# soasme/LTX-Video-GPUPoor

Measured on AMD Instinct MI355X. Metric: denoise-steps/sec + VAE-decode frames/sec, LTX-Video 768x512x97f at 1/8 GPU, higher is better.
Workload: dtype bf16

## Files before the change

### include/ltxmi.h

```cpp
#ifndef LTXMI_H
#define LTXMI_H

#include <stddef.h>
#include <stdint.h>

#ifdef __cplusplus
extern "C" {
#endif

typedef enum ltxmi_status {
    LTXMI_OK = 0,
    LTXMI_ERR_INVALID_ARG = -1,
    LTXMI_ERR_UNSUPPORTED = -2,
    LTXMI_ERR_LAUNCH = -3
} ltxmi_status;

const char* ltxmi_version(void);
const char* ltxmi_last_error(void);
const char* ltxmi_arch(void);

typedef enum ltxmi_epilogue {
    LTXMI_EPI_NONE = 0,
    LTXMI_EPI_GELU_TANH = 1,
    LTXMI_EPI_SILU = 2,
    LTXMI_EPI_GATE_RESIDUAL = 3
} ltxmi_epilogue;

typedef struct ltxmi_gemm_args {
    const void* A;  int64_t lda;
    const void* W;  int64_t ldw;
    const void* bias;
    void*       C;  int64_t ldc;
    int32_t M, N, K;
    int32_t epilogue;
    const void* residual; int64_t ldr;
    const void* gate_table;
    const void* gate_temb;
    int64_t     gate_ld;
    int32_t     rows_per_group;
    int32_t     algo;
    float*      rowsumsq; int32_t rowsumsq_cols; int64_t rowsumsq_ld;
    int32_t     a_kblock; int64_t a_kblock_stride;
} ltxmi_gemm_args;

int ltxmi_gemm_bf16(const ltxmi_gemm_args* args, void* stream);
int ltxmi_gemm_kernel_id(const ltxmi_gemm_args* args);

typedef enum ltxmi_norm_kind { LTXMI_NORM_RMS = 0, LTXMI_NORM_LAYER = 1 } ltxmi_norm_kind;

int ltxmi_norm_modulate_bf16(const void* x, int64_t ldx, void* y, int64_t ldy,
                             int32_t rows, int32_t D, float eps, int32_t kind,
                             const void* scale_table, const void* scale_temb,
// ... 161 lines not shown
```

### ltx-video-gpupoor_amd/csrc/api.hip

```cpp
#include <stdarg.h>
#include <string.h>

#include "common.h"

namespace ltxmi {

static thread_local char g_err[512] = "";

void set_error(const char* fmt, ...) {
    va_list ap;
    va_start(ap, fmt);
    vsnprintf(g_err, sizeof(g_err), fmt, ap);
    va_end(ap);
}

int check_launch(const char* what) {
    const hipError_t e = hipGetLastError();
    if (e != hipSuccess) {
        set_error("%s: launch failed: %s", what, hipGetErrorString(e));
        return LTXMI_ERR_LAUNCH;
    }
    return LTXMI_OK;
}

// ... 6 lines not shown
    const bool tracked = dev >= 0 && dev < 64;
    const unsigned long long bit = tracked ? (1ull << dev) : 0ull;
    if (tracked && (__atomic_load_n(done, __ATOMIC_ACQUIRE) & bit)) return LTXMI_OK;
    const hipError_t e = hipFuncSetAttribute(kernel, hipFuncAttributeMaxDynamicSharedMemorySize, bytes);
    if (e != hipSuccess) {
        set_error("%s: cannot reserve %d bytes of LDS: %s", what, bytes, hipGetErrorString(e));
        return LTXMI_ERR_LAUNCH;
    }
    if (tracked) __atomic_fetch_or(done, bit, __ATOMIC_RELEASE);
    return LTXMI_OK;
}

int device_cu_count(const char* what) {
    static int cus[64] = {};
    int dev = 0;
    if (hipGetDevice(&dev) != hipSuccess) {
        set_error("%s: cannot query the current device", what);
        return -1;
    }
    const bool tracked = dev >= 0 && dev < 64;
    if (tracked) {
        const int c = __atomic_load_n(&cus[dev], __ATOMIC_ACQUIRE);
        if (c > 0) return c;
    }
    int n = 0;
    if (hipDeviceGetAttribute(&n, hipDeviceAttributeMultiprocessorCount, dev) != hipSuccess || n <= 0) {
        set_error("%s: cannot query the CU count of device %d", what, dev);
        return -1;
    }
    if (tracked) __atomic_store_n(&cus[dev], n, __ATOMIC_RELEASE);
    return n;
}

}

extern "C" const char* ltxmi_version(void) { return "ltxmi 0.9.0"; }
extern "C" const char* ltxmi_last_error(void) { return ltxmi::g_err; }
extern "C" const char* ltxmi_arch(void) { return "gfx950"; }
```

### ltx-video-gpupoor_amd/csrc/attention_cross.hip

```cpp
#include <type_traits>

#include "attention.h"

namespace ltxmi {

namespace cross {

#ifndef LTXMI_XATTN_STAGGER
#define LTXMI_XATTN_STAGGER 32
#endif

constexpr int DH = 64;
constexpr int KV_TILE = 64;
constexpr int MAX_TILES = 4;
constexpr int ROW_BYTES = DH * 2;
constexpr int TILE_BYTES = KV_TILE * DH * 2;
constexpr int K_OFF = 0, V_OFF = MAX_TILES * TILE_BYTES, BIAS_OFF = 2 * MAX_TILES * TILE_BYTES;
constexpr int SCR_OFF = BIAS_OFF + MAX_TILES * KV_TILE * 16;
constexpr int SCR_BYTES = 32 * 64;
constexpr int QW_OFF = SCR_OFF + 4 * SCR_BYTES;
constexpr int SMEM = QW_OFF + DH * 2;
constexpr int ROWS_PER_IT = 128;
constexpr float LOG2E = 1.4426950408889634f;

__device__ __forceinline__ int k_swz(int row) { return (row >> 1) & 7; }

template <int NT>
__global__ __launch_bounds__(256, 2) void attn_cross_kernel(AttnParams p, int groups, int rows_per_group, int stagger_from) {
    extern __shared__ __attribute__((aligned(16))) char smem[];
    const int tid = threadIdx.x;
    const int lane = tid & 63;
    const int wave = __builtin_amdgcn_readfirstlane(tid >> 6);
    const int r = lane & 31, hh = lane >> 5;

    const int work = xcd_work_id();
    const int bh = work / groups, grp = work % groups;
    const int b = bh / p.H, head = bh % p.H;
    const int row_begin = grp * rows_per_group;
    const int row_end = min(p.Lq, row_begin + rows_per_group);
    if (row_begin >= row_end) return;
    const int n_it = (row_end - row_begin + ROWS_PER_IT - 1) / ROWS_PER_IT;

    const uint16_t* qb = p.q + (int64_t)b * p.q_sb + head * DH;
    const uint16_t* kb_ = p.k + (int64_t)b * p.k_sb + head * DH;
    const uint16_t* vb = p.v + (int64_t)b * p.v_sb + head * DH;
    uint16_t* ob = p.o + (int64_t)b * p.o_sb + head * DH;
    constexpr int nt = NT;

    {
        u32x4 kreg[NT][2], vreg[NT][2];
#pragma unroll
        for (int t = 0; t < NT; ++t) {
#pragma unroll
                for (int i = 0; i < 2; ++i) {
                    const int c = tid + 256 * i;
                    int key = t * KV_TILE + (c >> 3);
                    key = key < p.Lk ? key : p.Lk - 1;
                    kreg[t][i] = *(const u32x4*)(kb_ + (int64_t)key * p.k_sl + (c & 7) * 8);
                    vreg[t][i] = *(const u32x4*)(vb + (int64_t)key * p.v_sl + (c & 7) * 8);
                }
            }
// ... 16 lines not shown
                    *(u32x4*)(smem + V_OFF + t * TILE_BYTES + ((key >> 3) * 2 + (dc >> 2)) * 512 + (key & 7) * 64 + (dc & 3) * 16) = vreg[t][i];
                }
            }
    }
    if (p.q_on_load() && tid < 8) *(u32x4*)(smem + QW_OFF + tid * 16) = *(const u32x4*)(p.q_w + head * DH + tid * 8);
    __syncthreads();

    const int k_rd0 = r * ROW_BYTES, k_rd1 = (32 + r) * ROW_BYTES;
    const int k_sw0 = k_swz(r);
    const int g16 = lane >> 4, i16 = lane & 15;
    const int v_rd = (4 * (g16 >> 1) + (i16 >> 2)) * 64 + (16 * (g16 & 1) + 4 * (i16 & 3)) * 2;
    bf16x8 ones;
    {
        const bool on = ((lane & 15) == 0 && ((lane >> 4) & 1) == 0) || ((lane & 15) == 1 && ((lane >> 4) & 1) == 1);
#pragma unroll
        for (int e = 0; e < 8; ++e) ones[e] = on ? (__bf16)1.0f : (__bf16)0.0f;
    }
    const float c = p.scale_log2e;
    char* scr = smem + SCR_OFF + wave * SCR_BYTES;

    bf16x8 qraw[4], qf[4];
    float q_rstd = 0.f;
    int q_ld = 0;
    auto load_q = [&](int it) {
        const int row = row_begin + it * ROWS_PER_IT + wave * 32 + r;
        q_ld = row < p.Lq ? row : p.Lq - 1;
#pragma unroll
        for (int s = 0; s < 4; ++s) qraw[s] = *(const bf16x8*)(qb + (int64_t)q_ld * p.q_sl + 16 * s + 8 * hh);
        if (p.q_on_load()) q_rstd = p.q_row_rstd(b, q_ld, p.H * DH);
    };
    auto finish_q = [&]() {
        if (p.q_on_load()) {
            const int64_t trow = (int64_t)b * p.rope_sb + (int64_t)q_ld * p.rope_sl;
#pragma unroll
            for (int s = 0; s < 4; ++s) {
                const bf16x8 wv = *(const bf16x8*)(smem + QW_OFF + (16 * s + 8 * hh) * 2);
                float o[8];
#pragma unroll
                for (int e = 0; e < 8; ++e) o[e] = (float)qraw[s][e] * q_rstd * (float)wv[e];
                if (p.rope_cos) {
                    const int col = head * DH + 16 * s + 8 * hh;
                    const bf16x8 cv = *(const bf16x8*)(p.rope_cos + trow + col), sv = *(const bf16x8*)(p.rope_sin + trow + col);
#pragma unroll
                    for (int e = 0; e < 8; e += 2) {
                        const float r0 = o[e] * (float)cv[e] - o[e + 1] * (float)sv[e];
                        const float r1 = o[e + 1] * (float)cv[e + 1] + o[e] * (float)sv[e + 1];
                        o[e] = r0;
                        o[e + 1] = r1;
                    }
                }
#pragma unroll
                for (int e = 0; e < 8; ++e) qf[s][e] = (__bf16)o[e];
            }
        } else {
#pragma unroll
            for (int s = 0; s < 4; ++s) qf[s] = qraw[s];
        }
    };
    load_q(0);
    finish_q();
    if (n_it > 1) load_q(1);
    if (blockIdx.x >= (unsigned)stagger_from) __builtin_amdgcn_s_sleep(LTXMI_XATTN_STAGGER);

    for (int it = 0; it < n_it; ++it) {
        const int q0 = row_begin + it * ROWS_PER_IT + wave * 32;

        constexpr int NG = 2 * NT;
        f32x16 sT[NG];
        bf16x8 kfr[5];
        bf16x8 qaug;
        {
            uint32_t w0 = hh == 0 ? 0x3f803f80u : 0u, w1 = 0u;
            asm volatile("" : "+v"(w0), "+v"(w1));
            const u32x4 w = {w0, w1, w1, w1};
            qaug = __builtin_bit_cast(bf16x8, w);
        }
        auto read_k1 = [&](int g, int j) {
            if (j == 0) {
                kfr[0] = *(const bf16x8*)(smem + BIAS_OFF + (32 * g + r) * 16);
            } else {
                const char* ks = smem + K_OFF + (g >> 1) * TILE_BYTES + ((g & 1) ? k_rd1 : k_rd0);
                kfr[j] = *(const bf16x8*)(ks + (((2 * (j - 1) + hh) ^ k_sw0) << 4));
            }
        };
        auto max3 = [](float a, float b2, float c3) { return fmaxf(fmaxf(a, b2), c3); };
        float mt = -INFINITY;
        auto group_max = [&](int g) {
            const f32x16& x = sT[g];
            const float a = max3(x[0], x[1], x[2]), b2 = max3(x[3], x[4], x[5]), c2 = max3(x[6], x[7], x[8]);
            const float d2 = max3(x[9], x[10], x[11]), e2 = max3(x[12], x[13], x[14]);
            mt = max3(max3(a, b2, c2), max3(d2, e2, x[15]), mt);
            asm volatile("" : "+v"(mt));
        };
#pragma unroll
        for (int j = 0; j < 5; ++j) read_k1(0, j);
#pragma unroll
        for (int g = 0; g < NG; ++g) {
#pragma unroll
            for (int j = 0; j < 5; ++j) {
                if (j == 0) {
                    const f32x16 z16 = {0.f, 0.f, 0.f, 0.f, 0.f, 0.f, 0.f, 0.f, 0.f, 0.f, 0.f, 0.f, 0.f, 0.f, 0.f, 0.f};
                    sT[g] = __builtin_amdgcn_mfma_f32_32x32x16_bf16(kfr[0], qaug, z16, 0, 0, 0);
                } else {
                    sT[g] = __builtin_amdgcn_mfma_f32_32x32x16_bf16(kfr[j], qf[j - 1], sT[g], 0, 0, 0);
                }
                if (g + 1 < NG) read_k1(g + 1, j);
                __builtin_amdgcn_sched_barrier(0);
            }
            if (g >= 1) group_max(g - 1);
        }
        if (it + 1 < n_it) finish_q();
        if (it + 2 < n_it) load_q(it + 2);
        group_max(NG - 1);
        mt = attn_lane_half_max(mt);
        const float nmc = -mt * c;

        f32x16 oT[2];
        f32x4 lT;
        const f32x16 z16 = {0.f, 0.f, 0.f, 0.f, 0.f, 0.f, 0.f, 0.f, 0.f, 0.f, 0.f, 0.f, 0.f, 0.f, 0.f, 0.f};
        const f32x4 z4 = {0.f, 0.f, 0.f, 0.f};
        auto read_v = [&](int t, int sp, bf16x8 (&dst)[2]) {
            const char* vs = smem + V_OFF + t * TILE_BYTES + v_rd;
#pragma unroll
            for (int d = 0; d < 2; ++d)
                dst[d] = attn_vt_fragment<DH>(vs + (2 * sp * 2 + d) * 512);
        };
        auto make_p = [&](int t, int sp2, bf16x8& dst) {
            const f32x16& x = sT[2 * t + (sp2 >> 1)];
            const f32x2 c2v = {c, c}, m2v = {nmc, nmc};
#pragma unroll
            for (int e = 0; e < 8; e += 2) {
                const f32x2 y = f32x2{x[8 * (sp2 & 1) + e], x[8 * (sp2 & 1) + e + 1]} * c2v + m2v;
                dst[e] = (__bf16)fast_exp2(y[0]);
                dst[e + 1] = (__bf16)fast_exp2(y[1]);
            }
            asm volatile("" : "+v"(dst));
        };
        bf16x8 pfr[2][4], vfr[2][2];
#pragma unroll
        for (int sp = 0; sp < 4; ++sp) make_p(0, sp, pfr[0][sp]);
        read_v(0, 0, vfr[0]);
#pragma unroll
        for (int t = 0; t < NT; ++t) {
#pragma unroll
            for (int sp = 0; sp < 4; ++sp) {
                const int st = 4 * t + sp;
                if (st + 1 < 4 * NT) read_v((st + 1) >> 2, (st + 1) & 3, vfr[(st + 1) & 1]);
                const bf16x8& pf = pfr[t & 1][sp];
                lT = __builtin_amdgcn_mfma_f32_16x16x32_bf16(ones, pf, st == 0 ? z4 : lT, 0, 0, 0);
                oT[0] = __builtin_amdgcn_mfma_f32_32x32x16_bf16(vfr[st & 1][0], pf, st == 0 ? z16 : oT[0], 0, 0, 0);
                oT[1] = __builtin_amdgcn_mfma_f32_32x32x16_bf16(vfr[st & 1][1], pf, st == 0 ? z16 : oT[1], 0, 0, 0);
                if (t + 1 < NT) make_p(t + 1, sp, pfr[(t + 1) & 1][sp]);
                __builtin_amdgcn_sched_barrier(0);
            }
        }

        const float l0 = __shfl(lT[0], r & 15, 64), l1v = __shfl(lT[1], r & 15, 64);
        const float lrow = (r & 16) ? l1v : l0;
        const float inv = 1.0f / lrow;
        if (p.lse != nullptr) {
            if (hh == 0 && q0 + r < row_end) p.store_lse(b, head, q0 + r, -nmc, lrow, -nmc / c <= ATTN_ROW_REMOVED);
        }
#pragma unroll
        for (int d = 0; d < 2; ++d) {
#pragma unroll
            for (int g = 0; g < 4; ++g) {
                u32x2 w;
                w[0] = pack_bf16(oT[d][4 * g + 0] * inv, oT[d][4 * g + 1] * inv);
                w[1] = pack_bf16(oT[d][4 * g + 2] * inv, oT[d][4 * g + 3] * inv);
                *(u32x2*)(scr + r * 64 + ((g ^ (r & 3)) << 4) + hh * 8) = w;
            }
#pragma unroll
            for (int t2 = 0; t2 < 2; ++t2) {
                const int row = t2 * 16 + (lane >> 2), chunk = lane & 3;
                const u32x4 w = *(const u32x4*)(scr + row * 64 + ((chunk ^ (row & 3)) << 4));
                if (q0 + row < row_end) *(u32x4*)(ob + p.o_row(q0 + row) + 32 * d + chunk * 8) = w;
            }
        }
    }
}

}

static_assert(cross::MAX_TILES * cross::KV_TILE == ATTN_CROSS_MAX_KEYS, "attn_select hands this kernel up to ATTN_CROSS_MAX_KEYS keys");

int launch_attn_cross(AttnParams p, hipStream_t stream) {
    const int n_cu = device_cu_count("ltxmi_attention_fwd_bf16");
    if (n_cu <= 0) return LTXMI_ERR_LAUNCH;
    const int slots = 2 * n_cu, bh = p.B * p.H;
    int groups = slots / bh;
    if (groups < 1) groups = 1;
    const int max_groups = (p.Lq + 2 * cross::ROWS_PER_IT - 1) / (2 * cross::ROWS_PER_IT);
    if (groups > max_groups) groups = max_groups;
    int rows = (p.Lq + groups - 1) / groups;
    rows = (rows + cross::ROWS_PER_IT - 1) / cross::ROWS_PER_IT * cross::ROWS_PER_IT;
    groups = (p.Lq + rows - 1) / rows;
    const int nt = (p.Lk + cross::KV_TILE - 1) / cross::KV_TILE;
#define LTXMI_XATTN_LAUNCH(N)                                                                                              \
    {                                                                                                                      \
        static unsigned long long lds_done = 0;                                                                            \
        return attn_launch(cross::attn_cross_kernel<N>, cross::SMEM, &lds_done, p, groups, stream, groups, rows, n_cu);    \
    }
    switch (nt) {
        case 1: LTXMI_XATTN_LAUNCH(1)
        case 2: LTXMI_XATTN_LAUNCH(2)
        case 3: LTXMI_XATTN_LAUNCH(3)
        default: LTXMI_XATTN_LAUNCH(4)
    }
#undef LTXMI_XATTN_LAUNCH
}

}
```

### ltx-video-gpupoor_amd/csrc/common.h

```cpp
#pragma once
#include <hip/hip_runtime.h>
#include <stdint.h>
#include <stdio.h>

#include <type_traits>

#include "../../include/ltxmi.h"

namespace ltxmi {

typedef __attribute__((ext_vector_type(8))) __bf16 bf16x8;
typedef __attribute__((ext_vector_type(4))) __bf16 bf16x4;
typedef __attribute__((ext_vector_type(4))) float f32x4;
typedef __attribute__((ext_vector_type(16))) float f32x16;
typedef __attribute__((ext_vector_type(4))) short s16x4;
typedef __attribute__((ext_vector_type(4))) uint32_t u32x4;
typedef __attribute__((ext_vector_type(2))) uint32_t u32x2;

typedef __attribute__((address_space(3))) void* lds_void_ptr;
typedef const __attribute__((address_space(1))) void* glb_void_ptr;

constexpr int WAVE = 64;

__device__ __forceinline__ float bf2f(uint16_t h) { return __uint_as_float(((uint32_t)h) << 16); }
// ... 24 lines not shown
    const f32x2 x = {a, b};
    const f32x2 u = x * x * f32x2{-0.10294324f, -0.10294324f} + f32x2{-2.30220820f, -2.30220820f};
    const f32x2 nz = x * u;
    const f32x2 d = f32x2{fast_exp2(nz[0]), fast_exp2(nz[1])} + f32x2{1.0f, 1.0f};
    const f32x2 r = x * f32x2{fast_rcp(d[0]), fast_rcp(d[1])};
    a = r[0];
    b = r[1];
}

__device__ __forceinline__ float wave_sum(float v) {
#pragma unroll
    for (int o = 32; o > 0; o >>= 1) v += __shfl_xor(v, o, 64);
    return v;
}

__device__ __forceinline__ int xcd_work_id() {
    const int nwg = gridDim.x, orig = blockIdx.x;
    const int xcd = orig & 7, q = nwg >> 3, r = nwg & 7;
    return (xcd < r ? xcd * (q + 1) : r * (q + 1) + (xcd - r) * q) + (orig >> 3);
}

__device__ __forceinline__ void glds16(const void* gsrc, void* lds_wave_base) {
    __builtin_amdgcn_global_load_lds((glb_void_ptr)gsrc, (lds_void_ptr)lds_wave_base, 16, 0, 0);
}

__device__ __forceinline__ void blds16(__amdgpu_buffer_rsrc_t rsrc, void* lds_wave_base, uint32_t voff, int soff) {
    __builtin_amdgcn_raw_ptr_buffer_load_lds(rsrc, (lds_void_ptr)lds_wave_base, 16, (int)voff, soff, 0, 0);
}

void set_error(const char* fmt, ...);
int check_launch(const char* what);
int reserve_lds(const void* kernel, int bytes, unsigned long long* done, const char* what);
int device_cu_count(const char* what);
template <int E> using epi_t = std::integral_constant<int, E>;
template <auto Kernel, class Params>
int launch_with_lds(const Params& p, dim3 grid, dim3 block, int lds_bytes, hipStream_t stream, const char* what) {
    static unsigned long long lds_done = 0;
    if (const int rc = reserve_lds((const void*)Kernel, lds_bytes, &lds_done, what)) return rc;
    hipLaunchKernelGGL(Kernel, grid, block, lds_bytes, stream, p);
    return check_launch(what);
}

}

#define LTXMI_REQUIRE(cond, code, ...)          \
    do {                                        \
        if (!(cond)) {                          \
            ltxmi::set_error(__VA_ARGS__);      \
            return (code);                      \
        }                                       \
    } while (0)
```

### ltx-video-gpupoor_amd/csrc/rowops.hip

```cpp
#include "common.h"

namespace ltxmi {

constexpr int ROWS_PER_WG = 4;

struct Chunk {
    float v[8];
};
__device__ __forceinline__ Chunk load_chunk(const uint16_t* p) {
    const u32x4 w = *(const u32x4*)p;
    Chunk c;
#pragma unroll
    for (int i = 0; i < 4; ++i) {
        c.v[2 * i] = bf_lo(w[i]);
        c.v[2 * i + 1] = bf_hi(w[i]);
    }
    return c;
}
__device__ __forceinline__ void store_chunk(uint16_t* p, const Chunk& c) {
    u32x4 w;
#pragma unroll
    for (int i = 0; i < 4; ++i) w[i] = pack_bf16(c.v[2 * i], c.v[2 * i + 1]);
    *(u32x4*)p = w;
}
// ... 22 lines not shown
                else s2 += c[j].v[e] * c[j].v[e];
            }
        }
    }
    float mean = 0.f;
    if (LAYER) {
        mean = wave_sum(s1) / D;
        s2 = 0.f;
#pragma unroll
        for (int j = 0; j < NCH; ++j) {
            if (lane + 64 * j < nchunk) {
#pragma unroll
                for (int e = 0; e < 8; ++e) {
                    const float d = c[j].v[e] - mean;
                    s2 += d * d;
                }
            }
        }
    }
    const float rstd = rsqrtf(wave_sum(s2) / D + eps);
    const int64_t g = (int64_t)(row / rows_per_group) * temb_ld;
    uint16_t* yr = y + (int64_t)row * ldy;
#pragma unroll
    for (int j = 0; j < NCH; ++j) {
        const int ch = lane + 64 * j;
        if (ch < nchunk) {
            const Chunk a = load_chunk(sc_tab + ch * 8), a2 = load_chunk(sc_temb + g + ch * 8);
            const Chunk b = load_chunk(sh_tab + ch * 8), b2 = load_chunk(sh_temb + g + ch * 8);
            Chunk o;
#pragma unroll
            for (int e = 0; e < 8; ++e)
                o.v[e] = (c[j].v[e] - mean) * rstd * (1.0f + a.v[e] + a2.v[e]) + (b.v[e] + b2.v[e]);
            store_chunk(yr + ch * 8, o);
        }
    }
}

template <int NCH>
__global__ __launch_bounds__(256) void rmsnorm_rope_kernel(uint16_t* __restrict__ x, int64_t ldx, int rows, int D,
                                                           const uint16_t* __restrict__ w, float eps,
                                                           const uint16_t* __restrict__ cs,
                                                           const uint16_t* __restrict__ sn, int64_t ld_tab,
                                                           int rope_period, const float* __restrict__ side_ss,
                                                           int64_t side_ld, int side_n, float side_inv_d, float side_eps,
                                                           float* __restrict__ side_rstd) {
    const int lane = threadIdx.x & 63;
    const int row = blockIdx.x * ROWS_PER_WG + (threadIdx.x >> 6);
    if (row >= rows) return;
    if (side_ss) {
        float t = 0.f;
        for (int j = lane; j < side_n; j += 64) t += side_ss[(int64_t)row * side_ld + j];
        t = wave_sum(t);
        if (lane == 0) side_rstd[row] = rsqrtf(t * side_inv_d + side_eps);
    }
    const int nchunk = D >> 3;
    uint16_t* xr = x + (int64_t)row * ldx;
    Chunk c[NCH];
    float s2 = 0.f;
#pragma unroll
    for (int j = 0; j < NCH; ++j) {
        const int ch = lane + 64 * j;
        if (ch < nchunk) {
            c[j] = load_chunk(xr + ch * 8);
#pragma unroll
            for (int e = 0; e < 8; ++e) s2 += c[j].v[e] * c[j].v[e];
        }
// ... 202 lines not shown
            if (cs) {
                const Chunk co = load_chunk(cs + trow + c0), si = load_chunk(sn + trow + c0);
                Chunk r2, r3;
#pragma unroll
                for (int e = 0; e < 8; e += 2) {
                    r2.v[e] = oq.v[e] * co.v[e] - oq.v[e + 1] * si.v[e];
                    r2.v[e + 1] = oq.v[e + 1] * co.v[e + 1] + oq.v[e] * si.v[e + 1];
                    r3.v[e] = ok.v[e] * co.v[e] - ok.v[e + 1] * si.v[e];
                    r3.v[e + 1] = ok.v[e + 1] * co.v[e + 1] + ok.v[e] * si.v[e + 1];
                }
                oq = r2;
                ok = r3;
            }
            store_chunk(dst, oq);
            store_chunk(dst + Dp, ok);
            *(u32x4*)(dst + 2 * Dp) = *(const u32x4*)(xr + 2 * D + c0);
        }
    }
}

static inline int nch_for(int D) { return D <= 512 ? 1 : (D <= 2048 ? 4 : 16); }

}

using namespace ltxmi;

#define DISPATCH_NCH(D, CALL)                  \
    switch (nch_for(D)) {                      \
        case 1: { constexpr int NCH = 1; CALL; } break;   \
        case 4: { constexpr int NCH = 4; CALL; } break;   \
        default: { constexpr int NCH = 16; CALL; } break; \
    }

extern "C" int ltxmi_norm_modulate_bf16(const void* x, int64_t ldx, void* y, int64_t ldy, int32_t rows, int32_t D,
                                        float eps, int32_t kind, const void* scale_table, const void* scale_temb,
                                        const void* shift_table, const void* shift_temb, int64_t temb_ld,
                                        int32_t rows_per_group, void* stream) {
    LTXMI_REQUIRE(x && y && scale_table && scale_temb && shift_table && shift_temb, LTXMI_ERR_INVALID_ARG,
                  "ltxmi_norm_modulate_bf16: NULL argument");
    LTXMI_REQUIRE(rows > 0 && D > 0 && rows_per_group > 0, LTXMI_ERR_INVALID_ARG,
                  "ltxmi_norm_modulate_bf16: non-positive size rows=%d D=%d", rows, D);
    LTXMI_REQUIRE(D % 8 == 0 && D <= 8192 && ldx % 8 == 0 && ldy % 8 == 0 && temb_ld % 8 == 0, LTXMI_ERR_UNSUPPORTED,
                  "ltxmi_norm_modulate_bf16: D=%d must be a multiple of 8 and <= 8192 (strides multiples of 8)", D);
    LTXMI_REQUIRE(kind == LTXMI_NORM_RMS || kind == LTXMI_NORM_LAYER, LTXMI_ERR_INVALID_ARG,
                  "ltxmi_norm_modulate_bf16: bad kind %d", kind);
    const int grid = (rows + ROWS_PER_WG - 1) / ROWS_PER_WG;
    hipStream_t s = (hipStream_t)stream;
#define CALLK(L)                                                                                            \
    hipLaunchKernelGGL((norm_modulate_kernel<NCH, L>), dim3(grid), dim3(256), 0, s, (const uint16_t*)x, ldx, \
                       (uint16_t*)y, ldy, rows, D, eps, (const uint16_t*)scale_table,                       \
                       (const uint16_t*)scale_temb, (const uint16_t*)shift_table, (const uint16_t*)shift_temb, \
                       temb_ld, rows_per_group)
    if (kind == LTXMI_NORM_LAYER) {
        DISPATCH_NCH(D, CALLK(true))
    } else {
        DISPATCH_NCH(D, CALLK(false))
    }
#undef CALLK
    return check_launch("ltxmi_norm_modulate_bf16");
}

static int rmsnorm_rope_launch(void* x, int64_t ldx, int32_t rows, int32_t D, const void* weight, float eps,
                               const void* cos_tab, const void* sin_tab, int64_t ld_tab, int32_t rope_period,
                               const float* side_ss, int64_t side_ld, int32_t side_n, int32_t side_d, float side_eps,
                               float* side_rstd, void* stream);

__global__ __launch_bounds__(256) void rowsumsq_rstd_kernel(const float* __restrict__ ss, int64_t ld, int n, int rows, float inv_d,
                                                            float eps, float* __restrict__ out) {
    const int t = blockIdx.x * 256 + threadIdx.x;
    const int r = t >> 3, part = t & 7;
    float acc = 0.f;
    if (r < rows) {
        const float* p = ss + (int64_t)r * ld;
        if ((n & 3) == 0 && ((ld & 3) == 0) && (((uintptr_t)ss) & 15) == 0) {
            for (int j = 4 * part; j < n; j += 32) {
                const f32x4 v = *(const f32x4*)(p + j);
                acc += (v[0] + v[1]) + (v[2] + v[3]);
            }
        } else {
            for (int j = part; j < n; j += 8) acc += p[j];
// ... 130 lines not shown
```

### ltx-video-gpupoor_amd/ltxmi/_lib.py

```python
import ctypes
import os

import torch

_HERE = os.path.dirname(os.path.abspath(__file__))
LIB_PATH = os.environ.get("LTXMI_LIB") or os.path.join(_HERE, "libltxmi.so")

c_void_p, c_int, c_int64, c_float = ctypes.c_void_p, ctypes.c_int32, ctypes.c_int64, ctypes.c_float


class GemmArgs(ctypes.Structure):
    _fields_ = [("A", c_void_p), ("lda", c_int64), ("W", c_void_p), ("ldw", c_int64), ("bias", c_void_p),
                ("C", c_void_p), ("ldc", c_int64), ("M", c_int), ("N", c_int), ("K", c_int),
                ("epilogue", c_int), ("residual", c_void_p), ("ldr", c_int64), ("gate_table", c_void_p),
                ("gate_temb", c_void_p), ("gate_ld", c_int64), ("rows_per_group", c_int), ("algo", c_int),
                ("rowsumsq", c_void_p), ("rowsumsq_cols", c_int), ("rowsumsq_ld", c_int64),
                ("a_kblock", c_int), ("a_kblock_stride", c_int64)]


class AttnArgs(ctypes.Structure):
    _fields_ = [("q", c_void_p), ("q_stride_b", c_int64), ("q_stride_l", c_int64),
                ("k", c_void_p), ("k_stride_b", c_int64), ("k_stride_l", c_int64),
                ("v", c_void_p), ("v_stride_b", c_int64), ("v_stride_l", c_int64),
                ("o", c_void_p), ("o_stride_b", c_int64), ("o_stride_l", c_int64),
# ... 12 lines not shown
ATTN_MERGE_MAX = 8


class AttnMergeArgs(ctypes.Structure):
    _fields_ = [("n", c_int),
                ("o_part", c_void_p * ATTN_MERGE_MAX), ("o_part_stride_b", c_int64 * ATTN_MERGE_MAX),
                ("o_part_stride_l", c_int64 * ATTN_MERGE_MAX),
                ("lse_part", c_void_p * ATTN_MERGE_MAX), ("lse_part_stride_b", c_int64 * ATTN_MERGE_MAX),
                ("lse_part_stride_h", c_int64 * ATTN_MERGE_MAX),
                ("o", c_void_p), ("o_stride_b", c_int64), ("o_stride_l", c_int64),
                ("lse", c_void_p), ("lse_stride_b", c_int64), ("lse_stride_h", c_int64),
                ("B", c_int), ("H", c_int), ("Lq", c_int), ("head_dim", c_int)]


class Conv3dArgs(ctypes.Structure):
    _fields_ = [("x", c_void_p), ("w", c_void_p), ("bias", c_void_p), ("y", c_void_p),
                ("B", c_int), ("T", c_int), ("H", c_int), ("W", c_int), ("Cin", c_int), ("Cout", c_int),
                ("causal", c_int), ("pad_replicate", c_int), ("d2s", c_int), ("residual", c_void_p),
                ("res_channels", c_int), ("add", c_void_p),
                ("stride_t", c_int), ("stride_hw", c_int), ("tpad", c_int), ("out_T", c_int),
                ("kernel_t", c_int), ("time_pad_zeros", c_int), ("algo", c_int),
                ("post_norm", c_int), ("post_scale", c_void_p), ("post_shift", c_void_p), ("post_eps", c_float),
                ("y_norm", c_void_p), ("workspace", c_void_p), ("workspace_bytes", c_int64)]


class Conv3dRouteInfo(ctypes.Structure):
    _fields_ = [("route", c_int), ("epilogue", c_int), ("ksplit", c_int), ("swap_hw", c_int), ("finalize_blocks", c_int)]


SIGNATURES = {
    "ltxmi_version": (ctypes.c_char_p, []),
    "ltxmi_last_error": (ctypes.c_char_p, []),
    "ltxmi_arch": (ctypes.c_char_p, []),
    "ltxmi_gemm_bf16": (c_int, [ctypes.POINTER(GemmArgs), c_void_p]),
    "ltxmi_gemm_kernel_id": (c_int, [ctypes.POINTER(GemmArgs)]),
    "ltxmi_norm_modulate_bf16": (c_int, [c_void_p, c_int64, c_void_p, c_int64, c_int, c_int, c_float, c_int,
                                         c_void_p, c_void_p, c_void_p, c_void_p, c_int64, c_int, c_void_p]),
    "ltxmi_norm_modulate_f32in_bf16": (c_int, [c_void_p, c_int64, c_void_p, c_int64, c_int, c_int, c_float, c_int,
                                               c_void_p, c_void_p, c_void_p, c_void_p, c_int64, c_int, c_void_p]),
    "ltxmi_gate_residual_f32": (c_int, [c_void_p, c_int64, c_void_p, c_int64, c_int, c_int, c_void_p, c_void_p, c_int64,
                                        c_int, c_int, c_void_p, c_int64, c_void_p]),
    "ltxmi_rmsnorm_rope_bf16": (c_int, [c_void_p, c_int64, c_int, c_int, c_void_p, c_float, c_void_p, c_void_p,
                                        c_int64, c_int, c_void_p]),
    "ltxmi_rmsnorm_rope_rstd_bf16": (c_int, [c_void_p, c_int64, c_int, c_int, c_void_p, c_float, c_void_p, c_void_p,
                                             c_int64, c_int, c_void_p, c_int64, c_int, c_int, c_float, c_void_p, c_void_p]),
    "ltxmi_rowsumsq_rstd_f32": (c_int, [c_void_p, c_int64, c_int, c_int, c_int, c_float, c_void_p, c_void_p]),
    "ltxmi_qkv_norm_rope_pack_bf16": (c_int, [c_void_p, c_int64, c_int, c_int, c_int, c_int, c_void_p, c_void_p, c_float,
                                              c_void_p, c_void_p, c_int64, c_int, c_void_p, c_void_p]),
    "ltxmi_attention_fwd_bf16": (c_int, [ctypes.POINTER(AttnArgs), c_void_p]),
    "ltxmi_attention_merge_bf16": (c_int, [ctypes.POINTER(AttnMergeArgs), c_void_p]),
    "ltxmi_attention_fuses_qnorm": (c_int, [c_int, c_int, c_int, c_int, c_int, c_int]),
    "ltxmi_attention_kernel_id": (c_int, [c_int, c_int, c_int, c_int, c_int, c_int, c_int64, c_int64]),
    "ltxmi_silu_bf16": (c_int, [c_void_p, c_void_p, c_int64, c_void_p]),
    "ltxmi_timestep_embedding_bf16": (c_int, [c_void_p, c_void_p, c_int, c_int, c_void_p]),
    "ltxmi_stg_blend_bf16": (c_int, [c_void_p, c_int64, c_void_p, c_int64, c_void_p, c_int, c_int, c_int, c_void_p]),
    "ltxmi_stg_blend_grouped_bf16": (c_int, [c_void_p, c_void_p, c_int64, c_int64, c_int64, c_void_p, c_int, c_int, c_int, c_int,
                                             c_void_p]),
    "ltxmi_conv3d_ndhwc_bf16": (c_int, [ctypes.POINTER(Conv3dArgs), c_void_p]),
    "ltxmi_conv3d_fuses_post_norm": (c_int, [ctypes.POINTER(Conv3dArgs)]),
    "ltxmi_conv3d_workspace_bytes": (c_int64, [ctypes.POINTER(Conv3dArgs)]),
    "ltxmi_conv3d_route": (c_int, [ctypes.POINTER(Conv3dArgs), ctypes.POINTER(Conv3dRouteInfo)]),
    "ltxmi_pixelnorm_ada_silu_bf16": (c_int, [c_void_p, c_void_p, c_int64, c_int, c_int64, c_void_p, c_void_p,
                                              c_int, c_float, c_void_p]),
    "ltxmi_add_bf16": (c_int, [c_void_p, c_void_p, c_void_p, c_int64, c_void_p]),
    "ltxmi_layernorm_affine_bf16": (c_int, [c_void_p, c_void_p, c_int64, c_int, c_void_p, c_void_p, c_float,
                                            c_void_p]),
# ... 51 lines not shown
```

### ltx-video-gpupoor_amd/ltxmi/ops.py

```python
import ctypes
import math

import torch

from . import _lib
from ._lib import lib, check

BF16 = torch.bfloat16

EPI_NONE, EPI_GELU_TANH, EPI_SILU, EPI_GATE_RESIDUAL = 0, 1, 2, 3
NORM_RMS, NORM_LAYER = 0, 1


def _stream():
    return ctypes.c_void_p(torch.cuda.current_stream().cuda_stream)


_watch = None
_events = {}


def watch_launches(keys):
    global _watch
    _watch = set(keys) if keys else None
# ... 96 lines not shown
        args.gate_temb = gate_temb.data_ptr()
        args.gate_ld = gate_temb.stride(0) if gate_temb.dim() == 2 else 0
    args.rows_per_group = rows_per_group
    args.algo = algo
    args.a_kblock, args.a_kblock_stride = a_kblock, a_kblock_stride
    if rowsumsq is not None:
        if rowsumsq.dtype != torch.float32 or rowsumsq.dim() != 2 or rowsumsq.shape[0] != M or rowsumsq.stride(1) != 1 \
                or rowsumsq.shape[1] * 64 < rowsumsq_cols:
            raise ValueError("ltxmi.gemm: rowsumsq must be fp32 [M, >= rowsumsq_cols/64]")
        args.rowsumsq, args.rowsumsq_cols, args.rowsumsq_ld = rowsumsq.data_ptr(), rowsumsq_cols, rowsumsq.stride(0)
    return args, out, M, N, K


def gemm(a, w, bias=None, out=None, epilogue=EPI_NONE, residual=None, gate_table=None, gate_temb=None,
         rows_per_group=1, algo=0, rowsumsq=None, rowsumsq_cols=0, a_kblock=0, a_kblock_stride=0):
    _chk_bf16(a, w, bias, out, residual, gate_table, gate_temb)
    args, out, M, N, K = _gemm_args(a, w, bias, out, epilogue, residual, gate_table, gate_temb, rows_per_group, algo,
                                    rowsumsq, rowsumsq_cols, a_kblock, a_kblock_stride, True)
    tok = _prof_begin(("gemm", M, N, K, epilogue))
    check(lib.ltxmi_gemm_bf16(ctypes.byref(args), _stream()), "ltxmi_gemm_bf16")
    _prof_end(tok)
    return out


GEMM_TILE128, GEMM_TILE256, GEMM_PERSISTENT256 = 0, 1, 2


def gemm_kernel_id(a, w, bias=None, out=None, epilogue=EPI_NONE, residual=None, gate_table=None, gate_temb=None,
                   rows_per_group=1, algo=0, rowsumsq=None, rowsumsq_cols=0, a_kblock=0, a_kblock_stride=0):
    _chk_bf16_any_device(a, w, bias, out, residual, gate_table, gate_temb)
    args = _gemm_args(a, w, bias, out, epilogue, residual, gate_table, gate_temb, rows_per_group, algo,
                      rowsumsq, rowsumsq_cols, a_kblock, a_kblock_stride, False)[0]
    return int(lib.ltxmi_gemm_kernel_id(ctypes.byref(args)))


def norm_modulate(x, out, eps, kind, scale_table, scale_temb, shift_table, shift_temb, rows_per_group):
    _chk_bf16(x, out, scale_table, scale_temb, shift_table, shift_temb)
    x2, rows, ldx = _rows(x)
    o2, _, ldy = _rows(out)
    D = x2.shape[1]
    if scale_temb.stride(0) != shift_temb.stride(0):
        raise ValueError("ltxmi.norm_modulate: scale/shift tables must share a row stride")
    check(lib.ltxmi_norm_modulate_bf16(_ptr(x2), ldx, _ptr(o2), ldy, rows, D, eps, kind,
                                       _ptr(scale_table), _ptr(scale_temb), _ptr(shift_table), _ptr(shift_temb),
                                       scale_temb.stride(0), rows_per_group, _stream()),
          "ltxmi_norm_modulate_bf16")
    return out


def _chk_f32(t, what):
    if t.dtype != torch.float32 or not t.is_cuda:
        raise TypeError(f"ltxmi.{what}: expected a CUDA float32 tensor, got {t.dtype} on {t.device}")


def norm_modulate_f32in(x, out, eps, kind, scale_table, scale_temb, shift_table, shift_temb, rows_per_group):
    _chk_f32(x, "norm_modulate_f32in")
    _chk_bf16(out, scale_table, scale_temb, shift_table, shift_temb)
    x2, rows, ldx = _rows(x)
    o2, orows, ldy = _rows(out)
    D = x2.shape[1]
    if orows != rows or o2.shape[1] != D:
        raise ValueError("ltxmi.norm_modulate_f32in: out must have x's rows and channels")
    if scale_temb.stride(0) != shift_temb.stride(0):
        raise ValueError("ltxmi.norm_modulate_f32in: scale/shift tables must share a row stride")
    check(lib.ltxmi_norm_modulate_f32in_bf16(_ptr(x2), ldx, _ptr(o2), ldy, rows, D, eps, kind,
                                             _ptr(scale_table), _ptr(scale_temb), _ptr(shift_table), _ptr(shift_temb),
# ... 575 lines not shown
```

Before: 16.19.

## Skip negligible cross-attention KV tiles and process multiple norm rows per wave

```diff
diff --git a/include/ltxmi.h b/include/ltxmi.h
--- a/include/ltxmi.h
+++ b/include/ltxmi.h
@@ -18,6 +18,14 @@
 const char* ltxmi_version(void);
 const char* ltxmi_last_error(void);
 const char* ltxmi_arch(void);
+
+typedef enum ltxmi_option {
+    LTXMI_OPT_XATTN_SKIP_DEAD_TILES = 0,
+    LTXMI_OPT_NORM_ROWS_PER_WAVE = 1,
+    LTXMI_OPTION_COUNT = 2
+} ltxmi_option;
+int ltxmi_set_option(int32_t option, int32_t value);
+int ltxmi_get_option(int32_t option);
 
 typedef enum ltxmi_epilogue {
     LTXMI_EPI_NONE = 0,
diff --git a/ltx-video-gpupoor_amd/csrc/api.hip b/ltx-video-gpupoor_amd/csrc/api.hip
--- a/ltx-video-gpupoor_amd/csrc/api.hip
+++ b/ltx-video-gpupoor_amd/csrc/api.hip
@@ -62,6 +62,25 @@
     return n;
 }
 
+static int g_options[LTXMI_OPTION_COUNT] = { 1,  2};
+
+int option(int which) { return __atomic_load_n(&g_options[which], __ATOMIC_RELAXED); }
+
+}
+
+extern "C" int ltxmi_set_option(int32_t option, int32_t value) {
+    LTXMI_REQUIRE(option >= 0 && option < LTXMI_OPTION_COUNT, LTXMI_ERR_INVALID_ARG, "ltxmi_set_option: unknown option %d", option);
+    if (option == LTXMI_OPT_XATTN_SKIP_DEAD_TILES)
+        LTXMI_REQUIRE(value == 0 || value == 1, LTXMI_ERR_INVALID_ARG, "ltxmi_set_option: skip_dead_tiles is 0 or 1, got %d", value);
+    if (option == LTXMI_OPT_NORM_ROWS_PER_WAVE)
+        LTXMI_REQUIRE(value == 1 || value == 2 || value == 4, LTXMI_ERR_INVALID_ARG,
+                      "ltxmi_set_option: norm rows per wave is 1, 2 or 4, got %d", value);
+    __atomic_store_n(&ltxmi::g_options[option], value, __ATOMIC_RELAXED);
+    return LTXMI_OK;
+}
+extern "C" int ltxmi_get_option(int32_t option) {
+    LTXMI_REQUIRE(option >= 0 && option < LTXMI_OPTION_COUNT, LTXMI_ERR_INVALID_ARG, "ltxmi_get_option: unknown option %d", option);
+    return ltxmi::option(option);
 }
 
 extern "C" const char* ltxmi_version(void) { return "ltxmi 0.9.0"; }
diff --git a/ltx-video-gpupoor_amd/csrc/attention_cross.hip b/ltx-video-gpupoor_amd/csrc/attention_cross.hip
--- a/ltx-video-gpupoor_amd/csrc/attention_cross.hip
+++ b/ltx-video-gpupoor_amd/csrc/attention_cross.hip
@@ -26,7 +26,8 @@
 __device__ __forceinline__ int k_swz(int row) { return (row >> 1) & 7; }
 
 template <int NT>
-__global__ __launch_bounds__(256, 2) void attn_cross_kernel(AttnParams p, int groups, int rows_per_group, int stagger_from) {
+__global__ __launch_bounds__(256, 2) void attn_cross_kernel(AttnParams p, int groups, int rows_per_group, int stagger_from,
+                                                           int skip_dead) {
     extern __shared__ __attribute__((aligned(16))) char smem[];
     const int tid = threadIdx.x;
     const int lane = tid & 63;
@@ -109,14 +110,16 @@
     auto finish_q = [&]() {
         if (p.q_on_load()) {
             const int64_t trow = (int64_t)b * p.rope_sb + (int64_t)q_ld * p.rope_sl;
+            int hh8 = 8 * hh;
+            asm volatile("" : "+v"(hh8));
 #pragma unroll
             for (int s = 0; s < 4; ++s) {
-                const bf16x8 wv = *(const bf16x8*)(smem + QW_OFF + (16 * s + 8 * hh) * 2);
+                const bf16x8 wv = *(const bf16x8*)(smem + QW_OFF + (16 * s + hh8) * 2);
                 float o[8];
 #pragma unroll
                 for (int e = 0; e < 8; ++e) o[e] = (float)qraw[s][e] * q_rstd * (float)wv[e];
                 if (p.rope_cos) {
-                    const int col = head * DH + 16 * s + 8 * hh;
+                    const int col = head * DH + 16 * s + hh8;
                     const bf16x8 cv = *(const bf16x8*)(p.rope_cos + trow + col), sv = *(const bf16x8*)(p.rope_sin + trow + col);
 #pragma unroll
                     for (int e = 0; e < 8; e += 2) {
@@ -152,21 +155,34 @@
             const u32x4 w = {w0, w1, w1, w1};
             qaug = __builtin_bit_cast(bf16x8, w);
         }
+        int k_sw = k_sw0;
+        asm volatile("" : "+v"(k_sw));
         auto read_k1 = [&](int g, int j) {
             if (j == 0) {
                 kfr[0] = *(const bf16x8*)(smem + BIAS_OFF + (32 * g + r) * 16);
             } else {
                 const char* ks = smem + K_OFF + (g >> 1) * TILE_BYTES + ((g & 1) ? k_rd1 : k_rd0);
-                kfr[j] = *(const bf16x8*)(ks + (((2 * (j - 1) + hh) ^ k_sw0) << 4));
+                kfr[j] = *(const bf16x8*)(ks + (((2 * (j - 1) + hh) ^ k_sw) << 4));
             }
         };
         auto max3 = [](float a, float b2, float c3) { return fmaxf(fmaxf(a, b2), c3); };
         float mt = -INFINITY;
+        float nmc0 = 0.f, tmax = 0.f;
+        uint32_t live_tiles = 1u;
         auto group_max = [&](int g) {
             const f32x16& x = sT[g];
             const float a = max3(x[0], x[1], x[2]), b2 = max3(x[3], x[4], x[5]), c2 = max3(x[6], x[7], x[8]);
             const float d2 = max3(x[9], x[10], x[11]), e2 = max3(x[12], x[13], x[14]);
-            mt = max3(max3(a, b2, c2), max3(d2, e2, x[15]), mt);
+            const float gm = fmaxf(max3(a, b2, c2), max3(d2, e2, x[15]));
+            mt = fmaxf(gm, mt);
+            if (NT > 1) {
+                if (g == 1) nmc0 = -attn_lane_half_max(mt) * c;
+                if (g >= 2 && !(g & 1)) tmax = gm;
+                if (g >= 2 && (g & 1)) {
+                    const bool live = !(__builtin_fmaf(c, fmaxf(tmax, gm), nmc0) < -150.0f);
+                    if (__builtin_amdgcn_ballot_w64(live) != 0) live_tiles |= 1u << (g >> 1);
+                }
+            }
             asm volatile("" : "+v"(mt));
         };
 #pragma unroll
@@ -192,6 +208,8 @@
         mt = attn_lane_half_max(mt);
         const float nmc = -mt * c;
 
+        const int n_live = (NT > 1 && skip_dead && c > 0.f) ? 32 - __builtin_clz(live_tiles) : NT;
+
         f32x16 oT[2];
         f32x4 lT;
         const f32x16 z16 = {0.f, 0.f, 0.f, 0.f, 0.f, 0.f, 0.f, 0.f, 0.f, 0.f, 0.f, 0.f, 0.f, 0.f, 0.f, 0.f};
@@ -217,19 +235,28 @@
 #pragma unroll
         for (int sp = 0; sp < 4; ++sp) make_p(0, sp, pfr[0][sp]);
         read_v(0, 0, vfr[0]);
-#pragma unroll
-        for (int t = 0; t < NT; ++t) {
-#pragma unroll
-            for (int sp = 0; sp < 4; ++sp) {
-                const int st = 4 * t + sp;
-                if (st + 1 < 4 * NT) read_v((st + 1) >> 2, (st + 1) & 3, vfr[(st + 1) & 1]);
-                const bf16x8& pf = pfr[t & 1][sp];
-                lT = __builtin_amdgcn_mfma_f32_16x16x32_bf16(ones, pf, st == 0 ? z4 : lT, 0, 0, 0);
-                oT[0] = __builtin_amdgcn_mfma_f32_32x32x16_bf16(vfr[st & 1][0], pf, st == 0 ? z16 : oT[0], 0, 0, 0);
-                oT[1] = __builtin_amdgcn_mfma_f32_32x32x16_bf16(vfr[st & 1][1], pf, st == 0 ? z16 : oT[1], 0, 0, 0);
-                if (t + 1 < NT) make_p(t + 1, sp, pfr[(t + 1) & 1][sp]);
-                __builtin_amdgcn_sched_barrier(0);
-            }
+        auto pv_tiles = [&](auto nl_tag) {
+            constexpr int NL = decltype(nl_tag)::value;
+#pragma unroll
+            for (int t = 0; t < NL; ++t) {
+#pragma unroll
+                for (int sp = 0; sp < 4; ++sp) {
+                    const int st = 4 * t + sp;
+                    if (st + 1 < 4 * NL) read_v((st + 1) >> 2, (st + 1) & 3, vfr[(st + 1) & 1]);
+                    const bf16x8& pf = pfr[t & 1][sp];
+                    lT = __builtin_amdgcn_mfma_f32_16x16x32_bf16(ones, pf, st == 0 ? z4 : lT, 0, 0, 0);
+                    oT[0] = __builtin_amdgcn_mfma_f32_32x32x16_bf16(vfr[st & 1][0], pf, st == 0 ? z16 : oT[0], 0, 0, 0);
+                    oT[1] = __builtin_amdgcn_mfma_f32_32x32x16_bf16(vfr[st & 1][1], pf, st == 0 ? z16 : oT[1], 0, 0, 0);
+                    if (t + 1 < NL) make_p(t + 1, sp, pfr[(t + 1) & 1][sp]);
+                    __builtin_amdgcn_sched_barrier(0);
+                }
+            }
+        };
+        switch (n_live) {
+            case 1: pv_tiles(epi_t<1>{}); break;
+            case 2: pv_tiles(epi_t<(NT >= 2 ? 2 : NT)>{}); break;
+            case 3: pv_tiles(epi_t<(NT >= 3 ? 3 : NT)>{}); break;
+            default: pv_tiles(epi_t<NT>{}); break;
         }
 
         const float l0 = __shfl(lT[0], r & 15, 64), l1v = __shfl(lT[1], r & 15, 64);
@@ -238,6 +265,8 @@
         if (p.lse != nullptr) {
             if (hh == 0 && q0 + r < row_end) p.store_lse(b, head, q0 + r, -nmc, lrow, -nmc / c <= ATTN_ROW_REMOVED);
         }
+        int scr_r = r * 64, scr_l = lane;
+        asm volatile("" : "+v"(scr_r), "+v"(scr_l));
 #pragma unroll
         for (int d = 0; d < 2; ++d) {
 #pragma unroll
@@ -245,11 +274,11 @@
                 u32x2 w;
                 w[0] = pack_bf16(oT[d][4 * g + 0] * inv, oT[d][4 * g + 1] * inv);
                 w[1] = pack_bf16(oT[d][4 * g + 2] * inv, oT[d][4 * g + 3] * inv);
-                *(u32x2*)(scr + r * 64 + ((g ^ (r & 3)) << 4) + hh * 8) = w;
+                *(u32x2*)(scr + scr_r + ((g ^ ((scr_r >> 6) & 3)) << 4) + hh * 8) = w;
             }
 #pragma unroll
             for (int t2 = 0; t2 < 2; ++t2) {
-                const int row = t2 * 16 + (lane >> 2), chunk = lane & 3;
+                const int row = t2 * 16 + (scr_l >> 2), chunk = scr_l & 3;
                 const u32x4 w = *(const u32x4*)(scr + row * 64 + ((chunk ^ (row & 3)) << 4));
                 if (q0 + row < row_end) *(u32x4*)(ob + p.o_row(q0 + row) + 32 * d + chunk * 8) = w;
             }
@@ -273,10 +302,11 @@
     rows = (rows + cross::ROWS_PER_IT - 1) / cross::ROWS_PER_IT * cross::ROWS_PER_IT;
     groups = (p.Lq + rows - 1) / rows;
     const int nt = (p.Lk + cross::KV_TILE - 1) / cross::KV_TILE;
+    const int skip = option(LTXMI_OPT_XATTN_SKIP_DEAD_TILES);
 #define LTXMI_XATTN_LAUNCH(N)                                                                                              \
     {                                                                                                                      \
         static unsigned long long lds_done = 0;                                                                            \
-        return attn_launch(cross::attn_cross_kernel<N>, cross::SMEM, &lds_done, p, groups, stream, groups, rows, n_cu);    \
+        return attn_launch(cross::attn_cross_kernel<N>, cross::SMEM, &lds_done, p, groups, stream, groups, rows, n_cu, skip); \
     }
     switch (nt) {
         case 1: LTXMI_XATTN_LAUNCH(1)
diff --git a/ltx-video-gpupoor_amd/csrc/common.h b/ltx-video-gpupoor_amd/csrc/common.h
--- a/ltx-video-gpupoor_amd/csrc/common.h
+++ b/ltx-video-gpupoor_amd/csrc/common.h
@@ -80,6 +80,7 @@
 int check_launch(const char* what);
 int reserve_lds(const void* kernel, int bytes, unsigned long long* done, const char* what);
 int device_cu_count(const char* what);
+int option(int which);
 template <int E> using epi_t = std::integral_constant<int, E>;
 template <auto Kernel, class Params>
 int launch_with_lds(const Params& p, dim3 grid, dim3 block, int lds_bytes, hipStream_t stream, const char* what) {
diff --git a/ltx-video-gpupoor_amd/csrc/rowops.hip b/ltx-video-gpupoor_amd/csrc/rowops.hip
--- a/ltx-video-gpupoor_amd/csrc/rowops.hip
+++ b/ltx-video-gpupoor_amd/csrc/rowops.hip
@@ -78,6 +78,103 @@
             for (int e = 0; e < 8; ++e)
                 o.v[e] = (c[j].v[e] - mean) * rstd * (1.0f + a.v[e] + a2.v[e]) + (b.v[e] + b2.v[e]);
             store_chunk(yr + ch * 8, o);
+        }
+    }
+}
+
+__device__ __forceinline__ Chunk widen_chunk(const u32x4& w) {
+    Chunk c;
+#pragma unroll
+    for (int i = 0; i < 4; ++i) {
+        c.v[2 * i] = bf_lo(w[i]);
+        c.v[2 * i + 1] = bf_hi(w[i]);
+    }
+    return c;
+}
+template <int NCH, int R, bool FULL>
+__global__ __launch_bounds__(256) void norm_modulate_rows_kernel(
+    const uint16_t* __restrict__ x, int64_t ldx, uint16_t* __restrict__ y, int64_t ldy, int rows, int D,
+    float eps, const uint16_t* __restrict__ sc_tab, const uint16_t* __restrict__ sc_temb,
+    const uint16_t* __restrict__ sh_tab, const uint16_t* __restrict__ sh_temb, int64_t temb_ld,
+    int rows_per_group) {
+    const int lane = threadIdx.x & 63;
+    const int wave = __builtin_amdgcn_readfirstlane(threadIdx.x >> 6);
+    const int row0 = (blockIdx.x * ROWS_PER_WG + wave) * R;
+    if (row0 >= rows) return;
+    const int nrow = min(R, rows - row0);
+    const int nchunk = D >> 3;
+    bool valid[NCH];
+    int off[NCH];
+#pragma unroll
+    for (int j = 0; j < NCH; ++j) {
+        valid[j] = FULL || lane + 64 * j < nchunk;
+        off[j] = valid[j] ? (lane + 64 * j) * 8 : 0;
+    }
+    u32x4 raw[NCH];
+    auto request = [&](int row) {
+        const uint16_t* xr = x + (int64_t)row * ldx;
+#pragma unroll
+        for (int j = 0; j < NCH; ++j) raw[j] = *(const u32x4*)(xr + off[j]);
+    };
+    request(row0);
+    u32x4 ta[NCH], tb[NCH], ta2[NCH], tb2[NCH];
+#pragma unroll
+    for (int j = 0; j < NCH; ++j) {
+        ta[j] = *(const u32x4*)(sc_tab + off[j]);
+        tb[j] = *(const u32x4*)(sh_tab + off[j]);
+    }
+    int grp = row0 / rows_per_group, in_grp = row0 - grp * rows_per_group;
+    bool fresh = true;
+#pragma unroll
+    for (int i = 0; i < R; ++i) {
+        if (i >= nrow) break;
+        const int row = row0 + i;
+        Chunk c[NCH];
+        float s2 = 0.f;
+#pragma unroll
+        for (int j = 0; j < NCH; ++j) {
+#pragma clang fp reassociate(off) contract(off)
+            c[j] = widen_chunk(raw[j]);
+            const float* v = c[j].v;
+            float sx = v[6] * v[6], sy = v[7] * v[7];
+            sx = __builtin_fmaf(v[2], v[2], sx);
+            sy = __builtin_fmaf(v[3], v[3], sy);
+            sx = __builtin_fmaf(v[4], v[4], sx);
+            sy = __builtin_fmaf(v[5], v[5], sy);
+            sx = __builtin_fmaf(v[j == 0 ? 1 : 0], v[j == 0 ? 1 : 0], sx);
+            sy = __builtin_fmaf(v[j == 0 ? 0 : 1], v[j == 0 ? 0 : 1], sy);
+            const float sc = sx + sy;
+            s2 = valid[j] ? (j == 0 ? sc : s2 + sc) : s2;
+        }
+        if (i + 1 < nrow) request(row + 1);
+        if (fresh) {
+            const int64_t g = (int64_t)grp * temb_ld;
+#pragma unroll
+            for (int j = 0; j < NCH; ++j) {
+                ta2[j] = *(const u32x4*)(sc_temb + g + off[j]);
+                tb2[j] = *(const u32x4*)(sh_temb + g + off[j]);
+            }
+            fresh = false;
+        }
+        const float rstd = rsqrtf(wave_sum(s2) / D + eps);
+        uint16_t* yr = y + (int64_t)row * ldy;
+#pragma unroll
+        for (int j = 0; j < NCH; ++j) {
+            asm volatile("" : "+v"(ta[j]), "+v"(ta2[j]), "+v"(tb[j]), "+v"(tb2[j]));
+            const Chunk a = widen_chunk(ta[j]), a2 = widen_chunk(ta2[j]);
+            const Chunk b = widen_chunk(tb[j]), b2 = widen_chunk(tb2[j]);
+            Chunk o;
+#pragma unroll
+            for (int e = 0; e < 8; ++e) {
+#pragma clang fp reassociate(off) contract(off)
+                o.v[e] = __builtin_fmaf(c[j].v[e] * rstd, (1.0f + a.v[e]) + a2.v[e], b.v[e] + b2.v[e]);
+            }
+            if (valid[j]) store_chunk(yr + off[j], o);
+        }
+        if (++in_grp == rows_per_group) {
+            in_grp = 0;
+            ++grp;
+            fresh = true;
         }
     }
 }
@@ -346,6 +443,9 @@
         default: { constexpr int NCH = 16; CALL; } break; \
     }
 
+#define DISPATCH_NCH4(D, CALL)                 \
+    if (nch_for(D) == 1) { constexpr int NCH = 1; CALL; } else { constexpr int NCH = 4; CALL; }
+
 extern "C" int ltxmi_norm_modulate_bf16(const void* x, int64_t ldx, void* y, int64_t ldy, int32_t rows, int32_t D,
                                         float eps, int32_t kind, const void* scale_table, const void* scale_temb,
                                         const void* shift_table, const void* shift_temb, int64_t temb_ld,
@@ -358,8 +458,22 @@
                   "ltxmi_norm_modulate_bf16: D=%d must be a multiple of 8 and <= 8192 (strides multiples of 8)", D);
     LTXMI_REQUIRE(kind == LTXMI_NORM_RMS || kind == LTXMI_NORM_LAYER, LTXMI_ERR_INVALID_ARG,
                   "ltxmi_norm_modulate_bf16: bad kind %d", kind);
-    const int grid = (rows + ROWS_PER_WG - 1) / ROWS_PER_WG;
+    const int rpw = (kind == LTXMI_NORM_RMS && nch_for(D) <= 4) ? option(LTXMI_OPT_NORM_ROWS_PER_WAVE) : 1;
+    const int grid = (rows + ROWS_PER_WG * rpw - 1) / (ROWS_PER_WG * rpw);
     hipStream_t s = (hipStream_t)stream;
+#define CALLR(R, F)                                                                                                 \
+    hipLaunchKernelGGL((norm_modulate_rows_kernel<NCH, R, F>), dim3(grid), dim3(256), 0, s, (const uint16_t*)x, ldx, \
+                       (uint16_t*)y, ldy, rows, D, eps, (const uint16_t*)scale_table,                               \
+                       (const uint16_t*)scale_temb, (const uint16_t*)shift_table, (const uint16_t*)shift_temb,       \
+                       temb_ld, rows_per_group)
+#define CALLRF(R)                                          \
+    if (D == 512 * NCH) { CALLR(R, true); } else { CALLR(R, false); }
+    if (rpw == 2 || rpw == 4) {
+        if (rpw == 2) { DISPATCH_NCH4(D, CALLRF(2)) } else { DISPATCH_NCH4(D, CALLRF(4)) }
+        return check_launch("ltxmi_norm_modulate_bf16");
+    }
+#undef CALLRF
+#undef CALLR
 #define CALLK(L)                                                                                            \
     hipLaunchKernelGGL((norm_modulate_kernel<NCH, L>), dim3(grid), dim3(256), 0, s, (const uint16_t*)x, ldx, \
                        (uint16_t*)y, ldy, rows, D, eps, (const uint16_t*)scale_table,                       \
diff --git a/ltx-video-gpupoor_amd/ltxmi/_lib.py b/ltx-video-gpupoor_amd/ltxmi/_lib.py
--- a/ltx-video-gpupoor_amd/ltxmi/_lib.py
+++ b/ltx-video-gpupoor_amd/ltxmi/_lib.py
@@ -68,6 +68,8 @@
     "ltxmi_version": (ctypes.c_char_p, []),
     "ltxmi_last_error": (ctypes.c_char_p, []),
     "ltxmi_arch": (ctypes.c_char_p, []),
+    "ltxmi_set_option": (c_int, [c_int, c_int]),
+    "ltxmi_get_option": (c_int, [c_int]),
     "ltxmi_gemm_bf16": (c_int, [ctypes.POINTER(GemmArgs), c_void_p]),
     "ltxmi_gemm_kernel_id": (c_int, [ctypes.POINTER(GemmArgs)]),
     "ltxmi_norm_modulate_bf16": (c_int, [c_void_p, c_int64, c_void_p, c_int64, c_int, c_int, c_float, c_int,
diff --git a/ltx-video-gpupoor_amd/ltxmi/ops.py b/ltx-video-gpupoor_amd/ltxmi/ops.py
--- a/ltx-video-gpupoor_amd/ltxmi/ops.py
+++ b/ltx-video-gpupoor_amd/ltxmi/ops.py
@@ -152,6 +152,23 @@
     args = _gemm_args(a, w, bias, out, epilogue, residual, gate_table, gate_temb, rows_per_group, algo,
                       rowsumsq, rowsumsq_cols, a_kblock, a_kblock_stride, False)[0]
     return int(lib.ltxmi_gemm_kernel_id(ctypes.byref(args)))
+
+
+OPT_XATTN_SKIP_DEAD_TILES, OPT_NORM_ROWS_PER_WAVE = 0, 1
+
+
+def set_option(option, value):
+    old = int(lib.ltxmi_get_option(option))
+    check(lib.ltxmi_set_option(option, int(value)), "ltxmi_set_option")
+    return old
+
+
+def set_xattn_skip_dead_tiles(on):
+    return bool(set_option(OPT_XATTN_SKIP_DEAD_TILES, 1 if on else 0))
+
+
+def set_norm_rows_per_wave(n):
+    return set_option(OPT_NORM_ROWS_PER_WAVE, n)
 
 
 def norm_modulate(x, out, eps, kind, scale_table, scale_temb, shift_table, shift_temb, rows_per_group):
```

Result: no change. 16.30, median of 6 (+0.7%).
